# alasdairtran/fourierflow

Measured on AMD Instinct MI355X. Metric: training-steps/sec (whole node), F-FNO 24L 64x64 torus (torus_li/markov/24_layers), higher is better.
Workload: dtype f32

## Files before the change

### fourierflow_amd/csrc/ffx.hip

```cpp
#include <algorithm>

#include "ffno_device.h"
#include "ffno.h"

#include <string.h>

namespace ffno {

constexpr int kFfRangeTarget = 4;

template <int C, int H, int CPW_ = 1>
struct FxCfg {
    static constexpr int CPW = CPW_;
    static constexpr int NW = H / (32 * CPW);
    static constexpr int NT = NW * 64;
    static constexpr int KS = C / 16;
    static constexpr int CTO = C / 32;
    static constexpr int NV = (32 * C / 4) / NT;
    static constexpr int G = CTO * 4;
    static constexpr int GPW = G / NW;
    static constexpr int PROW = 2 * C + 16;
    static constexpr int PPLANE = 32 * PROW;
    static constexpr int TROW = 64 + 16;
    static constexpr int TPLANE = C * TROW;
// ... 1 lines not shown
    static_assert(NV >= 1 && NV * NT * 4 == 32 * C, "tile staging map");
    static_assert(GPW >= 1 && GPW * NW == G, "output reduction map");
};

struct FxPackDesc {
    const float* src;
    u32x4* dst;
    int sh, sc, type, pad;
};

template <class S>
__global__ __launch_bounds__(256) void ffx_pack_kernel(const FxPackDesc* __restrict__ descs, int C, int H) {
    const FxPackDesc d = descs[blockIdx.y];
    const int KS = C / 16, CTO = C / 32, NW = H / 32;
    const int nfrag = d.type == 1 ? NW * KS : NW * CTO * 2;
    const int t = blockIdx.x * blockDim.x + threadIdx.x;
    if (t >= nfrag * 64) return;
    const int frag = t >> 6, lane = t & 63, j = lane & 31, half = lane >> 5;
    float v[8];
    if (d.type == 1) {
        const int w = frag / KS, st = frag % KS;
        for (int e = 0; e < 8; ++e) v[e] = d.src[(long)(32 * w + j) * d.sh + (long)(16 * st + 8 * half + e) * d.sc];
    } else {
        const int s2 = frag & 1, mt = (frag >> 1) % CTO, w = (frag >> 1) / CTO;
        for (int e = 0; e < 8; ++e)
            v[e] = d.src[(long)(32 * w + (e & 3) + 8 * (2 * s2 + (e >> 2)) + 4 * half) * d.sh + (long)(32 * mt + j) * d.sc];
    }
    const typename S::Frag f = S::split8(v[0], v[1], v[2], v[3], v[4], v[5], v[6], v[7]);
    FFNO_UNROLL
    for (int p = 0; p < S::NP; ++p) d.dst[(frag * S::NP + p) * 64 + lane] = S::plane(f, p);
}

__device__ __forceinline__ Bf3 load_frag(const u32x4* __restrict__ pk, int frag, int lane) {
    Bf3 f;
    f.hi = pk[(frag * 3 + 0) * 64 + lane];
    f.mid = pk[(frag * 3 + 1) * 64 + lane];
    f.lo = pk[(frag * 3 + 2) * 64 + lane];
    return f;
}

__device__ __forceinline__ uint32_t push_sign(uint32_t acc, uint32_t x) {
    return plat::shift_in_msb(acc, x);
}
__device__ __forceinline__ uint32_t bit_mask(uint32_t x, int b) {
    return plat::bit_to_mask(x, b);
}

__device__ __forceinline__ Bf3 lds_frag(const char* base, int plane_bytes, int off) {
    Bf3 f;
    f.hi = *reinterpret_cast<const u32x4*>(base + off);
    f.mid = *reinterpret_cast<const u32x4*>(base + plane_bytes + off);
    f.lo = *reinterpret_cast<const u32x4*>(base + 2 * plane_bytes + off);
    return f;
}

__device__ __forceinline__ void stage4(char* base, int plane_bytes, int off, float x, float y, float z, float w) {
    unsigned h0, m0, l0, h1, m1, l1;
    split3_pair(x, y, h0, m0, l0);
    split3_pair(z, w, h1, m1, l1);
    *reinterpret_cast<uint2*>(base + off) = make_uint2(h0, h1);
    *reinterpret_cast<uint2*>(base + plane_bytes + off) = make_uint2(m0, m1);
    *reinterpret_cast<uint2*>(base + 2 * plane_bytes + off) = make_uint2(l0, l1);
}

template <class S>
__device__ __forceinline__ typename S::Frag load_frag_s(const u32x4* __restrict__ pk, int frag, int lane) {
    typename S::Frag f;
    FFNO_UNROLL
    for (int p = 0; p < S::NP; ++p) S::set_plane(f, p, pk[(frag * S::NP + p) * 64 + lane]);
    return f;
}
template <class S>
__device__ __forceinline__ typename S::Frag lds_frag_s(const char* base, int plane_bytes, int off) {
    typename S::Frag f;
    FFNO_UNROLL
    for (int p = 0; p < S::NP; ++p) S::set_plane(f, p, *reinterpret_cast<const u32x4*>(base + p * plane_bytes + off));
    return f;
}
template <class S>
__device__ __forceinline__ void stage4_s(char* base, int plane_bytes, int off, float x, float y, float z, float w) {
    uint2 pl[S::NP];
    S::split4(x, y, z, w, pl);
    FFNO_UNROLL
    for (int p = 0; p < S::NP; ++p) *reinterpret_cast<uint2*>(base + p * plane_bytes + off) = pl[p];
}

template <int C, int H, bool BWD, class S, class ST = StF32>
__global__ __launch_bounds__((FxCfg<C, H>::NT)) void ffx_chain_kernel(const typename ST::T* __restrict__ in,
                                                                     const typename ST::T* __restrict__ in2,
                                                                     typename ST::T* sum_out,
                                                                     const typename ST::T* resid,
                                                                     const u32x4* __restrict__ pk1,
                                                                     const float* __restrict__ bias1,
                                                                     const u32x4* __restrict__ pk2,
                                                                     const float* __restrict__ bias2, typename ST::T* out,
                                                                     uint32_t* mask, int P, const unsigned* in_amax, unsigned* out_amax) {
    using F = FxCfg<C, H>;
    constexpr int NW = F::NW, KS = F::KS, CTO = F::CTO, NV = F::NV, G = F::G, GPW = F::GPW, CPW = F::CPW;
    __shared__ __attribute__((aligned(16))) char sp[2][S::NP * F::PPLANE];
    __shared__ __attribute__((aligned(16))) float part[2][NW * G * 64 * 4];
    __shared__ __attribute__((aligned(16))) float b1s[H];
    __shared__ float b2s[C];

    const int tid = threadIdx.x, lane = tid & 63, wave = tid >> 6;
    const int j = lane & 31, half = lane >> 5;
    const int ntiles = (P + 31) >> 5;
    const float gscale = (S::SCALED && in_amax) ? range_scale(*in_amax, 1, kFfRangeTarget) : 1.f;
    const float rgscale = 1.f / gscale;
    float omax = 0.f;
    __shared__ float rfold[NW];

    using Frag = typename S::Frag;
    Frag A1[CPW][KS], A2[CPW][CTO][2];
    FFNO_UNROLL
    for (int ch = 0; ch < CPW; ++ch) {
        const int q = wave * CPW + ch;
        FFNO_UNROLL
        for (int st = 0; st < KS; ++st) A1[ch][st] = load_frag_s<S>(pk1, q * KS + st, lane);
        FFNO_UNROLL
        for (int mt = 0; mt < CTO; ++mt) {
            FFNO_UNROLL
            for (int s2 = 0; s2 < 2; ++s2) A2[ch][mt][s2] = load_frag_s<S>(pk2, (q * CTO + mt) * 2 + s2, lane);
        }
    }
    if (!BWD) {
        for (int e = tid; e < H; e += F::NT) b1s[e] = bias1[e] * gscale;
        for (int e = tid; e < C; e += F::NT) b2s[e] = bias2[e];
    }

    float4 nS[NV];
    typename ST::Raw4 pA[NV], pB[NV];
    auto gload_raw = [&](int tile) {
        FFNO_UNROLL
        for (int v = 0; v < NV; ++v) {
            const int f = tid + v * F::NT;
            const long px = (long)tile * 32 + f / (C / 4);
            pA[v] = pB[v] = ST::zero4();
            if (px < P) {
                const long off = px * C + 4 * (f % (C / 4));
                pA[v] = ST::ldr4(in + off);
                if (in2) pB[v] = ST::ldr4(in2 + off);
            }
        }
    };
    auto consume = [&](int tile) {
        FFNO_UNROLL
        for (int v = 0; v < NV; ++v) {
            nS[v] = ST::w4(pA[v]);
            if (in2) {
                const float4 b = ST::w4(pB[v]);
                nS[v].x += b.x, nS[v].y += b.y, nS[v].z += b.z, nS[v].w += b.w;
                nS[v] = st_rnd4<ST>(nS[v]);
                if (sum_out) {
                    const int f = tid + v * F::NT;
                    const long px = (long)tile * 32 + f / (C / 4);
                    if (px < P) ST::st4(sum_out + px * C + 4 * (f % (C / 4)), nS[v]);
                }
            }
            if (S::SCALED) nS[v].x *= gscale, nS[v].y *= gscale, nS[v].z *= gscale, nS[v].w *= gscale;
        }
    };
    auto stage = [&](int buf) {
        FFNO_UNROLL
        for (int v = 0; v < NV; ++v) {
            const int f = tid + v * F::NT;
            stage4_s<S>(sp[buf], F::PPLANE, (f / (C / 4)) * F::PROW + (f % (C / 4)) * 8, nS[v].x, nS[v].y, nS[v].z, nS[v].w);
        }
    };
    typename ST::Raw4 rres[GPW], rnext[GPW];
    auto rload = [&](int tile) {
        const long px = (long)tile * 32 + j;
        FFNO_UNROLL
        for (int u = 0; u < GPW; ++u) {
            const int gi = wave * GPW + u;
            rnext[u] = ST::zero4();
            if (!BWD && resid && px < P)
                rnext[u] = ST::ldr4(resid + px * C + 32 * (gi >> 2) + 8 * (gi & 3) + 4 * half);
        }
    };
    auto reduce = [&](int tile, int buf) {
        const long px = (long)tile * 32 + j;
        FFNO_UNROLL
        for (int u = 0; u < GPW; ++u) {
            const int gi = wave * GPW + u;
            float4 acc = *reinterpret_cast<const float4*>(&part[buf][((0 * G + gi) * 64 + lane) * 4]);
            FFNO_UNROLL
            for (int w = 1; w < NW; ++w) {
                const float4 t = *reinterpret_cast<const float4*>(&part[buf][((w * G + gi) * 64 + lane) * 4]);
                acc.x += t.x;
                acc.y += t.y;
                acc.z += t.z;
                acc.w += t.w;
            }
            const int c0 = 32 * (gi >> 2) + 8 * (gi & 3) + 4 * half;
            if (S::SCALED) acc.x *= rgscale, acc.y *= rgscale, acc.z *= rgscale, acc.w *= rgscale;
            if (!BWD) {
                const float4 rr = ST::w4(rres[u]);
                acc.x += b2s[c0] + rr.x;
                acc.y += b2s[c0 + 1] + rr.y;
                acc.z += b2s[c0 + 2] + rr.z;
                acc.w += b2s[c0 + 3] + rr.w;
            }
            if (px < P) {
                ST::st4(out + px * C + c0, acc);
                acc = st_rnd4<ST>(acc);
                omax = fmaxf(fmaxf(omax, fmaxf(fabsf(acc.x), fabsf(acc.y))), fmaxf(fabsf(acc.z), fabsf(acc.w)));
            }
        }
    };

    if ((int)blockIdx.x < ntiles) {
        gload_raw(blockIdx.x);
        consume(blockIdx.x);
        stage(0);
        if ((int)(blockIdx.x + gridDim.x) < ntiles) gload_raw(blockIdx.x + gridDim.x);
    }
    uint32_t bits_next = 0;
    if (BWD && (int)blockIdx.x < ntiles)
        bits_next = reinterpret_cast<const uint16_t*>(mask)[((long)blockIdx.x * NW + wave) * 64 + lane];
    __syncthreads();

    const bool early = wave < NW / 2 || NW == 1;
    int buf = 0, prev = -1;
    for (int tile = blockIdx.x; tile < ntiles; tile += gridDim.x, buf ^= 1) {
        const int nt = tile + gridDim.x, nt2 = nt + gridDim.x;
        if (nt < ntiles) consume(nt);
        rload(tile);
        static_assert(CPW == 1, "one 16-bit sign word per (tile, wave, lane)");
        uint16_t* mp = mask ? reinterpret_cast<uint16_t*>(mask) + ((long)tile * NW + wave) * 64 + lane : nullptr;
        uint32_t bits = 0;
        if (BWD) {
            bits = bits_next;
            if (nt < ntiles) bits_next = reinterpret_cast<const uint16_t*>(mask)[((long)nt * NW + wave) * 64 + lane];
        }
        if (nt2 < ntiles) gload_raw(nt2);

        f32x16 d[CPW];
        {
            f32x16 dc[CPW];
            FFNO_UNROLL
            for (int ch = 0; ch < CPW; ++ch) d[ch] = zero16(), dc[ch] = zero16();
            FFNO_UNROLL
            for (int st = 0; st < KS; ++st) {
                const Frag b = lds_frag_s<S>(sp[buf], F::PPLANE, j * F::PROW + 32 * st + 16 * half);
                FFNO_UNROLL
                for (int ch = 0; ch < CPW; ++ch) S::mma(A1[ch][st], b, d[ch], dc[ch]);
            }
            FFNO_UNROLL
            for (int ch = 0; ch < CPW; ++ch) S::fold(d[ch], dc[ch]);
        }
        if (early && prev >= 0) reduce(prev, buf ^ 1);
        f32x16 o[CTO], oc[CTO];
        FFNO_UNROLL
        for (int mt = 0; mt < CTO; ++mt) o[mt] = zero16(), oc[mt] = zero16();
        FFNO_UNROLL
        for (int ch = 0; ch < CPW; ++ch) {
            if (BWD) {
                FFNO_UNROLL
                for (int r = 0; r < 16; ++r) d[ch][r] = u2f(f2u(d[ch][r]) & bit_mask(bits, 15 - r));
            } else {
                FFNO_UNROLL
                for (int g = 0; g < 4; ++g) {
                    const float4 bv = *reinterpret_cast<const float4*>(&b1s[32 * (wave * CPW + ch) + 8 * g + 4 * half]);
                    const float bb[4] = {bv.x, bv.y, bv.z, bv.w};
                    FFNO_UNROLL
                    for (int i = 0; i < 4; ++i) {
                        const float v = fmaxf(d[ch][4 * g + i] + bb[i], 0.f);
                        d[ch][4 * g + i] = v;
                        bits = push_sign(bits, 0u - f2u(v));
                    }
                }
            }
            Frag hb[2];
            hb[0] = S::split8(d[ch][0], d[ch][1], d[ch][2], d[ch][3], d[ch][4], d[ch][5], d[ch][6], d[ch][7]);
            hb[1] = S::split8(d[ch][8], d[ch][9], d[ch][10], d[ch][11], d[ch][12], d[ch][13], d[ch][14], d[ch][15]);
            FFNO_UNROLL
            for (int mt = 0; mt < CTO; ++mt) {
                S::mma(A2[ch][mt][0], hb[0], o[mt], oc[mt]);
                S::mma(A2[ch][mt][1], hb[1], o[mt], oc[mt]);
            }
        }
        FFNO_UNROLL
        for (int mt = 0; mt < CTO; ++mt) S::fold(o[mt], oc[mt]);
        if (!BWD && mp) *mp = (uint16_t)bits;
        FFNO_UNROLL
        for (int mt = 0; mt < CTO; ++mt) {
            FFNO_UNROLL
            for (int g = 0; g < 4; ++g)
                *reinterpret_cast<float4*>(&part[buf][(((wave * G) + mt * 4 + g) * 64 + lane) * 4]) =
                    make_float4(o[mt][4 * g], o[mt][4 * g + 1], o[mt][4 * g + 2], o[mt][4 * g + 3]);
        }
        if (!early && prev >= 0) reduce(prev, buf ^ 1);
        FFNO_UNROLL
        for (int u = 0; u < GPW; ++u) rres[u] = rnext[u];
        if (nt < ntiles) stage(buf ^ 1);
        prev = tile;
        __syncthreads();
    }
    if (prev >= 0) reduce(prev, buf ^ 1);
    if (out_amax) range_fold(omax, rfold, NW, out_amax);
}

template <int C, int H, bool BWD, class ST = StF32>
__global__ __launch_bounds__(512) FFNO_WAVES_PER_SIMD(2) void ffw_chain_kernel(const typename ST::T* __restrict__ in,
                                                                              const typename ST::T* __restrict__ in2,
                                                                              typename ST::T* sum_out,
                                                                              const typename ST::T* resid,
                                                                              const u32x4* __restrict__ pk1,
                                                                              const float* __restrict__ bias1,
                                                                              const u32x4* __restrict__ pk2,
                                                                              const float* __restrict__ bias2,
                                                                              typename ST::T* out, uint32_t* mask, int P,
                                                                              const unsigned* in_amax, unsigned* out_amax) {
    using S = SplitHf2;
    constexpr int NCH = H / 32, KS = C / 16, CTO = C / 32, NWV = 8;
    constexpr int NF1 = NCH * KS, NF2 = NCH * CTO * 2;
    constexpr int SROW = 20;
    FFNO_DYN_SMEM(smem);
    u32x4* w1 = reinterpret_cast<u32x4*>(smem);
    u32x4* w2 = w1 + NF1 * 2 * 64;
    float* b1s = reinterpret_cast<float*>(w2 + NF2 * 2 * 64);
    float* b2s = b1s + H;
    float* stg_all = b2s + C;
    __shared__ float rfold[NWV];

    const int tid = threadIdx.x, lane = tid & 63, wave = tid >> 6;
    const int j = lane & 31, half = lane >> 5;
    const int ntiles = (P + 31) >> 5;
    const float gscale = in_amax ? range_scale(*in_amax, 1, kFfRangeTarget) : 1.f;
    const float rgscale = 1.f / gscale;
    float omax = 0.f;

    for (int i = tid; i < NF1 * 2 * 64; i += NWV * 64) w1[i] = pk1[i];
    for (int i = tid; i < NF2 * 2 * 64; i += NWV * 64) w2[i] = pk2[i];
    if (!BWD) {
        for (int e = tid; e < H; e += NWV * 64) b1s[e] = bias1[e] * gscale;
        for (int e = tid; e < C; e += NWV * 64) b2s[e] = bias2[e];
    }
    __syncthreads();

    float* stg = stg_all + wave * (32 * SROW);
    const int mrow = lane >> 2, mq = lane & 3;
    float* stg_m0 = stg + mrow * SROW + 4 * mq;
    float* stg_o = stg + j * SROW + 8 * half;
    const uint16_t* mrd = reinterpret_cast<const uint16_t*>(mask);
    uint16_t* mwr = reinterpret_cast<uint16_t*>(mask);
    FFNO_NOUNROLL
    for (int tile = (int)blockIdx.x * NWV + wave; tile < ntiles; tile += (int)gridDim.x * NWV) {
        long mpx[2];
        bool mok[2];
        long moff[2];
        FFNO_UNROLL
        for (int i = 0; i < 2; ++i) {
            mpx[i] = (long)tile * 32 + 16 * i + mrow;
            mok[i] = mpx[i] < P;
            moff[i] = (mok[i] ? mpx[i] : (long)P - 1) * C + 4 * mq;
        }
        typename ST::Raw4 ra[KS][2], rb[KS][2];
        FFNO_UNROLL
        for (int st = 0; st < KS; ++st) {
            FFNO_UNROLL
            for (int i = 0; i < 2; ++i) ra[st][i] = ST::ldr4(in + moff[i] + 16 * st);
        }
        if (in2) {
            FFNO_UNROLL
            for (int st = 0; st < KS; ++st) {
                FFNO_UNROLL
                for (int i = 0; i < 2; ++i) rb[st][i] = ST::ldr4(in2 + moff[i] + 16 * st);
            }
        }
        typename ST::Raw4 rres[KS][2];
        uint32_t mw[NCH / 2];
        if (!BWD) {
            if (resid) {
                FFNO_UNROLL
                for (int st = 0; st < KS; ++st) {
                    FFNO_UNROLL
                    for (int i = 0; i < 2; ++i) rres[st][i] = ST::ldr4(resid + moff[i] + 16 * st);
                }
            }
        } else {
            static_assert(NCH % 2 == 0, "sign words are held in pairs");
            FFNO_UNROLL
            for (int q = 0; q < NCH / 2; ++q)
                mw[q] = (uint32_t)mrd[((long)tile * NCH + 2 * q) * 64 + lane] |
                        ((uint32_t)mrd[((long)tile * NCH + 2 * q + 1) * 64 + lane] << 16);
        }
        Hf2 b[KS];
        FFNO_UNROLL
        for (int st = 0; st < KS; ++st) {
            FFNO_UNROLL
            for (int i = 0; i < 2; ++i) {
                float4 v = ST::w4(ra[st][i]);
                if (in2) {
                    const float4 t = ST::w4(rb[st][i]);
                    v.x += t.x, v.y += t.y, v.z += t.z, v.w += t.w;
                    v = st_rnd4<ST>(v);
                    if (sum_out && mok[i]) ST::st4(sum_out + moff[i] + 16 * st, v);
                }
                const float sc = mok[i] ? gscale : 0.f;
                v.x *= sc, v.y *= sc, v.z *= sc, v.w *= sc;
                *reinterpret_cast<float4*>(stg_m0 + 16 * i * SROW) = v;
            }
            plat::wave_sync();
            const float4 v0 = *reinterpret_cast<const float4*>(stg_o), v1 = *reinterpret_cast<const float4*>(stg_o + 4);
            plat::wave_sync();
            b[st] = split2_8(v0.x, v0.y, v0.z, v0.w, v1.x, v1.y, v1.z, v1.w);
        }
        f32x16 o[CTO], oc[CTO];
        FFNO_UNROLL
        for (int mt = 0; mt < CTO; ++mt) o[mt] = zero16(), oc[mt] = zero16();
        FFNO_NOUNROLL
        for (int ch = 0; ch < NCH; ++ch) {
            uint32_t bits = 0;
            if (BWD) {
                uint32_t w = mw[0];
                FFNO_UNROLL
                for (int q = 1; q < NCH / 2; ++q) w = (ch >> 1) == q ? mw[q] : w;
                bits = (ch & 1) ? (w >> 16) : (w & 0xffffu);
            }
            f32x16 d = zero16(), dc = zero16();
            FFNO_UNROLL
            for (int st = 0; st < KS; ++st) {
                Hf2 a;
                a.hi = w1[((ch * KS + st) * 2 + 0) * 64 + lane];
                a.lo = w1[((ch * KS + st) * 2 + 1) * 64 + lane];
                mfma_h2(a, b[st], d, dc);
            }
            S::fold(d, dc);
            if (BWD) {
                FFNO_UNROLL
                for (int r = 0; r < 16; ++r) d[r] = u2f(f2u(d[r]) & bit_mask(bits, 15 - r));
            } else {
                FFNO_UNROLL
                for (int g = 0; g < 4; ++g) {
                    const float4 bv = *reinterpret_cast<const float4*>(&b1s[32 * ch + 8 * g + 4 * half]);
                    const float bb[4] = {bv.x, bv.y, bv.z, bv.w};
                    FFNO_UNROLL
                    for (int i = 0; i < 4; ++i) {
                        const float v = fmaxf(d[4 * g + i] + bb[i], 0.f);
                        d[4 * g + i] = v;
                        bits = push_sign(bits, 0u - f2u(v));
                    }
                }
                if (mwr) mwr[((long)tile * NCH + ch) * 64 + lane] = (uint16_t)bits;
            }
            Hf2 hb[2];
            hb[0] = split2_8(d[0], d[1], d[2], d[3], d[4], d[5], d[6], d[7]);
            hb[1] = split2_8(d[8], d[9], d[10], d[11], d[12], d[13], d[14], d[15]);
            FFNO_UNROLL
            for (int mt = 0; mt < CTO; ++mt) {
                FFNO_UNROLL
                for (int s2 = 0; s2 < 2; ++s2) {
                    Hf2 a;
                    a.hi = w2[(((ch * CTO + mt) * 2 + s2) * 2 + 0) * 64 + lane];
                    a.lo = w2[(((ch * CTO + mt) * 2 + s2) * 2 + 1) * 64 + lane];
                    mfma_h2(a, hb[s2], o[mt], oc[mt]);
                }
            }
        }
        FFNO_UNROLL
        for (int mt = 0; mt < CTO; ++mt) {
            S::fold(o[mt], oc[mt]);
            FFNO_UNROLL
            for (int gp = 0; gp < 2; ++gp) {
                const int blk = 2 * mt + gp;
                FFNO_UNROLL
                for (int u = 0; u < 2; ++u) {
                    const int g = 2 * gp + u;
                    *reinterpret_cast<float4*>(stg + j * SROW + 8 * u + 4 * half) =
                        make_float4(o[mt][4 * g], o[mt][4 * g + 1], o[mt][4 * g + 2], o[mt][4 * g + 3]);
                }
                plat::wave_sync();
                float4 acc[2];
                FFNO_UNROLL
                for (int i = 0; i < 2; ++i) acc[i] = *reinterpret_cast<const float4*>(stg_m0 + 16 * i * SROW);
                plat::wave_sync();
                FFNO_UNROLL
                for (int i = 0; i < 2; ++i) {
                    const int c0 = 16 * blk + 4 * mq;
                    acc[i].x *= rgscale, acc[i].y *= rgscale, acc[i].z *= rgscale, acc[i].w *= rgscale;
                    if (!BWD) {
                        float4 rr = make_float4(0.f, 0.f, 0.f, 0.f);
                        if (resid) rr = ST::w4(rres[blk][i]);
                        acc[i].x += b2s[c0] + rr.x;
                        acc[i].y += b2s[c0 + 1] + rr.y;
                        acc[i].z += b2s[c0 + 2] + rr.z;
                        acc[i].w += b2s[c0 + 3] + rr.w;
                    }
                    if (mok[i]) {
                        ST::st4(out + moff[i] + 16 * blk, acc[i]);
                        const float4 t = st_rnd4<ST>(acc[i]);
                        omax = fmaxf(fmaxf(omax, fmaxf(fabsf(t.x), fabsf(t.y))), fmaxf(fabsf(t.z), fabsf(t.w)));
                    }
                }
            }
        }
    }
    if (out_amax) range_fold(omax, rfold, NWV, out_amax);
}

template <int C, int H, bool BWD, class S, class ST = StF32>
__global__ __launch_bounds__((FxCfg<C, H>::NT)) void ffx_chain_rs_kernel(const typename ST::T* __restrict__ in,
                                                                        const typename ST::T* __restrict__ in2,
                                                                        typename ST::T* sum_out,
                                                                        const typename ST::T* resid,
                                                                        const u32x4* __restrict__ pk1,
                                                                        const float* __restrict__ bias1,
                                                                        const u32x4* __restrict__ pk2,
                                                                        const float* __restrict__ bias2, typename ST::T* out,
                                                                        uint32_t* mask, int P, const unsigned* in_amax, unsigned* out_amax) {
    using F = FxCfg<C, H>;
    constexpr int NW = F::NW, KS = F::KS, CTO = F::CTO, G = F::G;
    constexpr int NWA = NW / 2;
    constexpr int NTA = NWA * 64;
    constexpr int NVA = (32 * C / 4) / NTA;
    constexpr int GPB = G / NWA;
    static_assert(NW >= 2 && NWA * 2 == NW && NVA * NTA * 4 == 32 * C && GPB * NWA == G, "role split");
    __shared__ __attribute__((aligned(16))) char sp[2][S::NP * F::PPLANE];
    __shared__ __attribute__((aligned(16))) float part[NW * G * 64 * 4];
    __shared__ __attribute__((aligned(16))) float b1s[H];
    __shared__ float b2s[C];

    const int tid = threadIdx.x, lane = tid & 63, wave = tid >> 6;
    const int j = lane & 31, half = lane >> 5;
    const int ntiles = (P + 31) >> 5;
    const float gscale = (S::SCALED && in_amax) ? range_scale(*in_amax, 1, kFfRangeTarget) : 1.f;
    const float rgscale = 1.f / gscale;
    float omax = 0.f;
    __shared__ float rfold[NW];
    const bool first = wave < NWA;
    const int rw = wave - NWA;

    using Frag = typename S::Frag;
    Frag A1[KS], A2[CTO][2];
    FFNO_UNROLL
    for (int st = 0; st < KS; ++st) A1[st] = load_frag_s<S>(pk1, wave * KS + st, lane);
    FFNO_UNROLL
    for (int mt = 0; mt < CTO; ++mt) {
        FFNO_UNROLL
        for (int s2 = 0; s2 < 2; ++s2) A2[mt][s2] = load_frag_s<S>(pk2, (wave * CTO + mt) * 2 + s2, lane);
    }
    if (!BWD) {
        for (int e = tid; e < H; e += F::NT) b1s[e] = bias1[e] * gscale;
        for (int e = tid; e < C; e += F::NT) b2s[e] = bias2[e];
    }

    float4 pS[NVA];
    typename ST::Raw4 qA[NVA], qB[NVA];
    static_assert(!ST::BF16 || (NVA == 2 && GPB == 2), "bf16 storage: 16-byte accesses pair two float4 groups");
    auto fmap = [&](int v) { return ST::BF16 ? (tid / (C / 8)) * (C / 4) + 2 * (tid % (C / 8)) + v : tid + v * NTA; };
    auto gload_raw = [&](int tile) {
        if constexpr (ST::BF16) {
            const int f = fmap(0);
            const long px = (long)tile * 32 + f / (C / 4);
            qA[0] = qA[1] = qB[0] = qB[1] = ST::zero4();
            if (px < P) {
                const long off = px * C + 4 * (f % (C / 4));
                const u32x4 a = *reinterpret_cast<const u32x4*>(in + off);
                qA[0] = make_uint2(a[0], a[1]), qA[1] = make_uint2(a[2], a[3]);
                if (in2) {
                    const u32x4 b = *reinterpret_cast<const u32x4*>(in2 + off);
                    qB[0] = make_uint2(b[0], b[1]), qB[1] = make_uint2(b[2], b[3]);
                }
            }
        } else {
            FFNO_UNROLL
            for (int v = 0; v < NVA; ++v) {
                const int f = fmap(v);
                const long px = (long)tile * 32 + f / (C / 4);
                qA[v] = qB[v] = ST::zero4();
                if (px < P) {
                    const long off = px * C + 4 * (f % (C / 4));
                    qA[v] = ST::ldr4(in + off);
                    if (in2) qB[v] = ST::ldr4(in2 + off);
                }
            }
        }
    };
    auto consume = [&](int tile) {
        FFNO_UNROLL
        for (int v = 0; v < NVA; ++v) {
            pS[v] = ST::w4(qA[v]);
            if (in2) {
                const float4 b = ST::w4(qB[v]);
                pS[v].x += b.x, pS[v].y += b.y, pS[v].z += b.z, pS[v].w += b.w;
                pS[v] = st_rnd4<ST>(pS[v]);
                const int f = fmap(v);
                const long px = (long)tile * 32 + f / (C / 4);
                if constexpr (!ST::BF16)
                    if (sum_out && px < P) ST::st4(sum_out + px * C + 4 * (f % (C / 4)), pS[v]);
            }
        }
        if constexpr (ST::BF16) {
            const int f = fmap(0);
            const long px = (long)tile * 32 + f / (C / 4);
            if (in2 && sum_out && px < P) {
                u32x4 w;
                w[0] = plat::pack_bf16(pS[0].x, pS[0].y), w[1] = plat::pack_bf16(pS[0].z, pS[0].w);
                w[2] = plat::pack_bf16(pS[1].x, pS[1].y), w[3] = plat::pack_bf16(pS[1].z, pS[1].w);
                *reinterpret_cast<u32x4*>(sum_out + px * C + 4 * (f % (C / 4))) = w;
            }
        }
        if (S::SCALED) {
            FFNO_UNROLL
            for (int v = 0; v < NVA; ++v) pS[v].x *= gscale, pS[v].y *= gscale, pS[v].z *= gscale, pS[v].w *= gscale;
        }
    };
    auto stage = [&](int buf) {
        FFNO_UNROLL
        for (int v = 0; v < NVA; ++v) {
            const int f = fmap(v);
            stage4_s<S>(sp[buf], F::PPLANE, (f / (C / 4)) * F::PROW + (f % (C / 4)) * 8, pS[v].x, pS[v].y, pS[v].z, pS[v].w);
        }
    };
    typename ST::Raw4 rres[GPB], rnext[GPB];
    const int c16 = 32 * ((rw * GPB) >> 2) + 8 * (((rw * GPB) & 3) + half);
    auto rload = [&](int tile) {
        const long px = (long)tile * 32 + j;
        if constexpr (ST::BF16) {
            rnext[0] = rnext[1] = ST::zero4();
            if (!BWD && resid && px < P) {
                const u32x4 a = *reinterpret_cast<const u32x4*>(resid + px * C + c16);
                rnext[0] = make_uint2(a[0], a[1]), rnext[1] = make_uint2(a[2], a[3]);
            }
            return;
        }
        FFNO_UNROLL
        for (int u = 0; u < GPB; ++u) {
            const int gi = rw * GPB + u;
            rnext[u] = ST::zero4();
            if (!BWD && resid && px < P)
                rnext[u] = ST::ldr4(resid + px * C + 32 * (gi >> 2) + 8 * (gi & 3) + 4 * half);
        }
    };
    auto reduce = [&](int tile) {
        const long px = (long)tile * 32 + j;
        if constexpr (ST::BF16) {
            plat::swap_halves(rres[0].x, rres[1].x);
            plat::swap_halves(rres[0].y, rres[1].y);
        }
        uint2 pk16[2];
        FFNO_UNROLL
        for (int u = 0; u < GPB; ++u) {
            const int gi = rw * GPB + u;
            float4 acc = *reinterpret_cast<const float4*>(&part[((0 * G + gi) * 64 + lane) * 4]);
            FFNO_UNROLL
            for (int w = 1; w < NW; ++w) {
                const float4 t = *reinterpret_cast<const float4*>(&part[((w * G + gi) * 64 + lane) * 4]);
                acc.x += t.x;
                acc.y += t.y;
                acc.z += t.z;
                acc.w += t.w;
            }
            const int c0 = 32 * (gi >> 2) + 8 * (gi & 3) + 4 * half;
            if (S::SCALED) acc.x *= rgscale, acc.y *= rgscale, acc.z *= rgscale, acc.w *= rgscale;
            if (!BWD) {
                const float4 rr = ST::w4(rres[u]);
                acc.x += b2s[c0] + rr.x;
                acc.y += b2s[c0 + 1] + rr.y;
                acc.z += b2s[c0 + 2] + rr.z;
                acc.w += b2s[c0 + 3] + rr.w;
            }
            if constexpr (ST::BF16) pk16[u & 1] = make_uint2(plat::pack_bf16(acc.x, acc.y), plat::pack_bf16(acc.z, acc.w));
            if (px < P) {
                if constexpr (!ST::BF16) ST::st4(out + px * C + c0, acc);
                acc = st_rnd4<ST>(acc);
                omax = fmaxf(fmaxf(omax, fmaxf(fabsf(acc.x), fabsf(acc.y))), fmaxf(fabsf(acc.z), fabsf(acc.w)));
            }
        }
        if constexpr (ST::BF16) {
            plat::swap_halves(pk16[0].x, pk16[1].x);
            plat::swap_halves(pk16[0].y, pk16[1].y);
            if (px < P) {
                u32x4 w;
                w[0] = pk16[0].x, w[1] = pk16[0].y, w[2] = pk16[1].x, w[3] = pk16[1].y;
                *reinterpret_cast<u32x4*>(out + px * C + c16) = w;
            }
        }
    };

    f32x16 d;
    Frag hb[2];
    uint32_t bits = 0, bits_next = 0;
    auto gemm1 = [&](int buf) {
        f32x16 dc = zero16();
        d = zero16();
        FFNO_UNROLL
        for (int st = 0; st < KS; ++st) {
            const Frag b = lds_frag_s<S>(sp[buf], F::PPLANE, j * F::PROW + 32 * st + 16 * half);
            S::mma(A1[st], b, d, dc);
        }
        S::fold(d, dc);
    };
    auto epilogue = [&](int tile) {
        uint16_t* mp = mask ? reinterpret_cast<uint16_t*>(mask) + ((long)tile * NW + wave) * 64 + lane : nullptr;
        if (BWD) {
            bits = bits_next;
            const int nt = tile + gridDim.x;
            if (nt < ntiles) bits_next = reinterpret_cast<const uint16_t*>(mask)[((long)nt * NW + wave) * 64 + lane];
            FFNO_UNROLL
            for (int r = 0; r < 16; ++r) d[r] = u2f(f2u(d[r]) & bit_mask(bits, 15 - r));
        } else {
            bits = 0;
            FFNO_UNROLL
            for (int g = 0; g < 4; ++g) {
                const float4 bv = *reinterpret_cast<const float4*>(&b1s[32 * wave + 8 * g + 4 * half]);
                const float bb[4] = {bv.x, bv.y, bv.z, bv.w};
                FFNO_UNROLL
                for (int i = 0; i < 4; ++i) {
                    const float v = fmaxf(d[4 * g + i] + bb[i], 0.f);
                    d[4 * g + i] = v;
                    bits = push_sign(bits, 0u - f2u(v));
                }
            }
            if (mp) *mp = (uint16_t)bits;
        }
        hb[0] = S::split8(d[0], d[1], d[2], d[3], d[4], d[5], d[6], d[7]);
        hb[1] = S::split8(d[8], d[9], d[10], d[11], d[12], d[13], d[14], d[15]);
    };
    auto gemm2 = [&]() {
        f32x16 o[CTO];
        FFNO_UNROLL
        for (int mt = 0; mt < CTO; ++mt) {
            f32x16 oc = zero16();
            o[mt] = zero16();
            S::mma(A2[mt][0], hb[0], o[mt], oc);
            S::mma(A2[mt][1], hb[1], o[mt], oc);
            S::fold(o[mt], oc);
        }
        FFNO_UNROLL
        for (int mt = 0; mt < CTO; ++mt) {
            FFNO_UNROLL
            for (int g = 0; g < 4; ++g)
                *reinterpret_cast<float4*>(&part[(((wave * G) + mt * 4 + g) * 64 + lane) * 4]) =
                    make_float4(o[mt][4 * g], o[mt][4 * g + 1], o[mt][4 * g + 2], o[mt][4 * g + 3]);
        }
    };

    const int t0 = blockIdx.x, gs = gridDim.x;
    if (first) {
        if (t0 < ntiles) {
            gload_raw(t0);
            consume(t0);
            stage(0);
        }
        if (t0 + gs < ntiles) {
            gload_raw(t0 + gs);
            consume(t0 + gs);
        }
        if (t0 + 2 * gs < ntiles) gload_raw(t0 + 2 * gs);
    } else if (t0 < ntiles) {
        rload(t0);
    }
    if (BWD && t0 < ntiles) bits_next = reinterpret_cast<const uint16_t*>(mask)[((long)t0 * NW + wave) * 64 + lane];
    __syncthreads();

    int buf = 0, prev = -1;
    for (int tile = t0; tile < ntiles; tile += gs, buf ^= 1) {
        const int nt = tile + gs;
        if (first) {
            gemm1(buf);
        } else {
            if (prev >= 0) reduce(prev);
            FFNO_UNROLL
            for (int u = 0; u < GPB; ++u) rres[u] = rnext[u];
            if (nt < ntiles) rload(nt);
        }
        __syncthreads();
        if (first)
            epilogue(tile);
        else
            gemm1(buf);
        __syncthreads();
        if (first)
            gemm2();
        else
            epilogue(tile);
        __syncthreads();
        if (first) {
            if (nt < ntiles) stage(buf ^ 1);
            if (nt + gs < ntiles) consume(nt + gs);
            if (nt + 2 * gs < ntiles) gload_raw(nt + 2 * gs);
        } else {
            gemm2();
        }
        prev = tile;
        __syncthreads();
    }
    if (!first && prev >= 0) reduce(prev);
    if (out_amax) range_fold(omax, rfold, NW, out_amax);
}

template <int C, int H, class S>
__global__ __launch_bounds__((FxCfg<C, H>::NT)) void ffx_wgrad_kernel(const float* __restrict__ s,
                                                                     const float* __restrict__ db,
                                                                     const u32x4* __restrict__ pk1,
                                                                     const float* __restrict__ bias1,
                                                                     const u32x4* __restrict__ pk2t,
                                                                     float* __restrict__ partial, int P, const unsigned* s_amax,
// ... 927 lines not shown
```

Before: 186.2.

## Prefetch next tile inputs and residual ahead of compute in ffw chain kernel

In the forward path of ffw_chain_kernel, the next tile's input loads are issued before the current tile's epilogue, and the residual load is moved to after staging so it overlaps the MFMA chain. The first tile's input is requested alongside the weight and bias copy into shared memory, which now goes through registers in one combined pass. The aim is to hide global-load latency behind compute. The cost is more live registers, which can lower occupancy or cause spills. Unconditional loads from fallback pointers add redundant memory traffic when in2 or resid is null, and __restrict__ is dropped from in and in2.

```diff
diff --git a/fourierflow_amd/csrc/ffx.hip b/fourierflow_amd/csrc/ffx.hip
--- a/fourierflow_amd/csrc/ffx.hip
+++ b/fourierflow_amd/csrc/ffx.hip
@@ -327,8 +327,7 @@
 }
 
 template <int C, int H, bool BWD, class ST = StF32>
-__global__ __launch_bounds__(512) FFNO_WAVES_PER_SIMD(2) void ffw_chain_kernel(const typename ST::T* __restrict__ in,
-                                                                              const typename ST::T* __restrict__ in2,
+__global__ __launch_bounds__(512) FFNO_WAVES_PER_SIMD(2) void ffw_chain_kernel(const typename ST::T* in, const typename ST::T* in2,
                                                                               typename ST::T* sum_out,
                                                                               const typename ST::T* resid,
                                                                               const u32x4* __restrict__ pk1,
@@ -356,60 +355,96 @@
     const float rgscale = 1.f / gscale;
     float omax = 0.f;
 
-    for (int i = tid; i < NF1 * 2 * 64; i += NWV * 64) w1[i] = pk1[i];
-    for (int i = tid; i < NF2 * 2 * 64; i += NWV * 64) w2[i] = pk2[i];
-    if (!BWD) {
-        for (int e = tid; e < H; e += NWV * 64) b1s[e] = bias1[e] * gscale;
-        for (int e = tid; e < C; e += NWV * 64) b2s[e] = bias2[e];
-    }
-    __syncthreads();
-
     float* stg = stg_all + wave * (32 * SROW);
     const int mrow = lane >> 2, mq = lane & 3;
     float* stg_m0 = stg + mrow * SROW + 4 * mq;
     float* stg_o = stg + j * SROW + 8 * half;
     const uint16_t* mrd = reinterpret_cast<const uint16_t*>(mask);
     uint16_t* mwr = reinterpret_cast<uint16_t*>(mask);
+
+    auto tile_rows = [&](int tile, long (&moff)[2], bool (&mok)[2]) {
+        FFNO_UNROLL
+        for (int i = 0; i < 2; ++i) {
+            const long mpx = (long)tile * 32 + 16 * i + mrow;
+            mok[i] = mpx < P;
+            moff[i] = (mok[i] ? mpx : (long)P - 1) * C + 4 * mq;
+        }
+    };
+    const typename ST::T* in2r = in2 ? in2 : in;
+    const typename ST::T* resr = resid ? resid : in;
+    typename ST::Raw4 ra[KS][2], rb[KS][2], rres[KS][2];
+    static_assert(NCH % 2 == 0, "sign words are held in pairs");
+    uint32_t mw[NCH / 2];
+    auto request_in = [&](int tile) {
+        long moff[2];
+        bool mok[2];
+        tile_rows(tile, moff, mok);
+        FFNO_UNROLL
+        for (int st = 0; st < KS; ++st) {
+            FFNO_UNROLL
+            for (int i = 0; i < 2; ++i) ra[st][i] = ST::ldr4(in + moff[i] + 16 * st);
+        }
+        if (BWD && !in2) return;
+        FFNO_UNROLL
+        for (int st = 0; st < KS; ++st) {
+            FFNO_UNROLL
+            for (int i = 0; i < 2; ++i) rb[st][i] = ST::ldr4(in2r + moff[i] + 16 * st);
+        }
+    };
+    auto request_resid = [&](int tile) {
+        long moff[2];
+        bool mok[2];
+        tile_rows(tile, moff, mok);
+        FFNO_UNROLL
+        for (int st = 0; st < KS; ++st) {
+            FFNO_UNROLL
+            for (int i = 0; i < 2; ++i) rres[st][i] = ST::ldr4(resr + moff[i] + 16 * st);
+        }
+    };
+    auto request_signs = [&](int tile) {
+        FFNO_UNROLL
+        for (int q = 0; q < NCH / 2; ++q)
+            mw[q] = (uint32_t)mrd[((long)tile * NCH + 2 * q) * 64 + lane] |
+                    ((uint32_t)mrd[((long)tile * NCH + 2 * q + 1) * 64 + lane] << 16);
+    };
+
+    constexpr int WPT = (NF1 + NF2) * 2 * 64 / (NWV * 64);
+    static_assert(WPT * NWV * 64 == (NF1 + NF2) * 2 * 64 && NF1 == NF2, "weight copy map");
+    static_assert(H + C <= NWV * 64 && 2 * (H + C) >= NWV * 64, "bias copy map");
+    const int tstep = (int)gridDim.x * NWV;
+    int tile = (int)blockIdx.x * NWV + wave;
+    if (BWD) {
+        for (int i = tid; i < NF1 * 2 * 64; i += NWV * 64) w1[i] = pk1[i];
+        for (int i = tid; i < NF2 * 2 * 64; i += NWV * 64) w2[i] = pk2[i];
+    } else {
+        u32x4 wreg[WPT];
+        FFNO_UNROLL
+        for (int q = 0; q < WPT; ++q) {
+            const int idx = tid + q * (NWV * 64);
+            wreg[q] = idx < NF1 * 2 * 64 ? pk1[idx] : pk2[idx - NF1 * 2 * 64];
+        }
+        const int be = tid < H + C ? tid : tid - (H + C);
+        const float v = *(be < H ? bias1 + be : bias2 + (be - H));
+        const float bv = be < H ? v * gscale : v;
+        FFNO_SCHED_PIN_VMEM();
+        const int t0 = tile < ntiles ? tile : ntiles - 1;
+        request_in(t0);
+        FFNO_SCHED_PIN_VMEM();
+        FFNO_UNROLL
+        for (int q = 0; q < WPT; ++q) w1[tid + q * (NWV * 64)] = wreg[q];
+        b1s[be] = bv;
+    }
+    __syncthreads();
+
     FFNO_NOUNROLL
-    for (int tile = (int)blockIdx.x * NWV + wave; tile < ntiles; tile += (int)gridDim.x * NWV) {
-        long mpx[2];
+    for (; tile < ntiles; tile += tstep) {
+        long moff[2];
         bool mok[2];
-        long moff[2];
-        FFNO_UNROLL
-        for (int i = 0; i < 2; ++i) {
-            mpx[i] = (long)tile * 32 + 16 * i + mrow;
-            mok[i] = mpx[i] < P;
-            moff[i] = (mok[i] ? mpx[i] : (long)P - 1) * C + 4 * mq;
-        }
-        typename ST::Raw4 ra[KS][2], rb[KS][2];
-        FFNO_UNROLL
-        for (int st = 0; st < KS; ++st) {
-            FFNO_UNROLL
-            for (int i = 0; i < 2; ++i) ra[st][i] = ST::ldr4(in + moff[i] + 16 * st);
-        }
-        if (in2) {
-            FFNO_UNROLL
-            for (int st = 0; st < KS; ++st) {
-                FFNO_UNROLL
-                for (int i = 0; i < 2; ++i) rb[st][i] = ST::ldr4(in2 + moff[i] + 16 * st);
-            }
-        }
-        typename ST::Raw4 rres[KS][2];
-        uint32_t mw[NCH / 2];
-        if (!BWD) {
-            if (resid) {
-                FFNO_UNROLL
-                for (int st = 0; st < KS; ++st) {
-                    FFNO_UNROLL
-                    for (int i = 0; i < 2; ++i) rres[st][i] = ST::ldr4(resid + moff[i] + 16 * st);
-                }
-            }
-        } else {
-            static_assert(NCH % 2 == 0, "sign words are held in pairs");
-            FFNO_UNROLL
-            for (int q = 0; q < NCH / 2; ++q)
-                mw[q] = (uint32_t)mrd[((long)tile * NCH + 2 * q) * 64 + lane] |
-                        ((uint32_t)mrd[((long)tile * NCH + 2 * q + 1) * 64 + lane] << 16);
+        tile_rows(tile, moff, mok);
+        const bool more = tile + tstep < ntiles;
+        if (BWD) {
+            request_in(tile);
+            request_signs(tile);
         }
         Hf2 b[KS];
         FFNO_UNROLL
@@ -431,6 +466,10 @@
             const float4 v0 = *reinterpret_cast<const float4*>(stg_o), v1 = *reinterpret_cast<const float4*>(stg_o + 4);
             plat::wave_sync();
             b[st] = split2_8(v0.x, v0.y, v0.z, v0.w, v1.x, v1.y, v1.z, v1.w);
+        }
+        if (!BWD) {
+            request_resid(tile);
+            FFNO_SCHED_PIN_VMEM();
         }
         f32x16 o[CTO], oc[CTO];
         FFNO_UNROLL
@@ -484,43 +523,56 @@
                 }
             }
         }
-        FFNO_UNROLL
-        for (int mt = 0; mt < CTO; ++mt) {
-            S::fold(o[mt], oc[mt]);
-            FFNO_UNROLL
-            for (int gp = 0; gp < 2; ++gp) {
-                const int blk = 2 * mt + gp;
+        auto epilogue = [&]() __attribute__((always_inline)) {
+            FFNO_UNROLL
+            for (int mt = 0; mt < CTO; ++mt) {
+                S::fold(o[mt], oc[mt]);
                 FFNO_UNROLL
-                for (int u = 0; u < 2; ++u) {
-                    const int g = 2 * gp + u;
-                    *reinterpret_cast<float4*>(stg + j * SROW + 8 * u + 4 * half) =
-                        make_float4(o[mt][4 * g], o[mt][4 * g + 1], o[mt][4 * g + 2], o[mt][4 * g + 3]);
-                }
-                plat::wave_sync();
-                float4 acc[2];
-                FFNO_UNROLL
-                for (int i = 0; i < 2; ++i) acc[i] = *reinterpret_cast<const float4*>(stg_m0 + 16 * i * SROW);
-                plat::wave_sync();
-                FFNO_UNROLL
-                for (int i = 0; i < 2; ++i) {
-                    const int c0 = 16 * blk + 4 * mq;
-                    acc[i].x *= rgscale, acc[i].y *= rgscale, acc[i].z *= rgscale, acc[i].w *= rgscale;
-                    if (!BWD) {
-                        float4 rr = make_float4(0.f, 0.f, 0.f, 0.f);
-                        if (resid) rr = ST::w4(rres[blk][i]);
-                        acc[i].x += b2s[c0] + rr.x;
-                        acc[i].y += b2s[c0 + 1] + rr.y;
-                        acc[i].z += b2s[c0 + 2] + rr.z;
-                        acc[i].w += b2s[c0 + 3] + rr.w;
+                for (int gp = 0; gp < 2; ++gp) {
+                    const int blk = 2 * mt + gp;
+                    FFNO_UNROLL
+                    for (int u = 0; u < 2; ++u) {
+                        const int g = 2 * gp + u;
+                        *reinterpret_cast<float4*>(stg + j * SROW + 8 * u + 4 * half) =
+                            make_float4(o[mt][4 * g], o[mt][4 * g + 1], o[mt][4 * g + 2], o[mt][4 * g + 3]);
                     }
-                    if (mok[i]) {
-                        ST::st4(out + moff[i] + 16 * blk, acc[i]);
-                        const float4 t = st_rnd4<ST>(acc[i]);
-                        omax = fmaxf(fmaxf(omax, fmaxf(fabsf(t.x), fabsf(t.y))), fmaxf(fabsf(t.z), fabsf(t.w)));
+                    plat::wave_sync();
+                    float4 acc[2];
+                    FFNO_UNROLL
+                    for (int i = 0; i < 2; ++i) acc[i] = *reinterpret_cast<const float4*>(stg_m0 + 16 * i * SROW);
+                    plat::wave_sync();
+                    FFNO_UNROLL
+                    for (int i = 0; i < 2; ++i) {
+                        const int c0 = 16 * blk + 4 * mq;
+                        acc[i].x *= rgscale, acc[i].y *= rgscale, acc[i].z *= rgscale, acc[i].w *= rgscale;
+                        if (!BWD) {
+                            float4 rr = make_float4(0.f, 0.f, 0.f, 0.f);
+                            if (resid) rr = ST::w4(rres[blk][i]);
+                            acc[i].x += b2s[c0] + rr.x;
+                            acc[i].y += b2s[c0 + 1] + rr.y;
+                            acc[i].z += b2s[c0 + 2] + rr.z;
+                            acc[i].w += b2s[c0 + 3] + rr.w;
+                        }
+                        if (mok[i]) {
+                            ST::st4(out + moff[i] + 16 * blk, acc[i]);
+                            const float4 t = st_rnd4<ST>(acc[i]);
+                            omax = fmaxf(fmaxf(omax, fmaxf(fabsf(t.x), fabsf(t.y))), fmaxf(fabsf(t.z), fabsf(t.w)));
+                        }
                     }
                 }
             }
-        }
+        };
+        if (BWD) {
+            epilogue();
+            continue;
+        }
+        if (!more) {
+            epilogue();
+            break;
+        }
+        request_in(tile + tstep);
+        FFNO_SCHED_PIN_VMEM();
+        epilogue();
     }
     if (out_amax) range_fold(omax, rfold, NWV, out_amax);
 }
```

Result: no change. 186.1 (median of 2 runs) (-0.0%).
